# Peacebeuponu94/lachain

Hardware: AMD Instinct MI355X
Metric: BLS12-381 TPKE decryption-share verifications/sec (batched VerifyShare, N=22 F=7) (higher is better)
Workload: dtype u32 (381-bit Montgomery, 12x32-bit limbs); 1 GPU; configs[1]: 1M TPKE decryption shares, N=22 F=7 validators, one MI355X per rank; ciphertexts_per_rank=47663, decryptors=22, degree=7, parallelism=shard1, decision_mismatches=0, batches_in_flight=4, hw_queues=4, hw_queues_env=4

## Files before the change

### include/lachain_bls.h

```cpp
#ifndef LACHAIN_BLS_H
#define LACHAIN_BLS_H
#include <stddef.h>
#include <stdint.h>
#ifdef __cplusplus
extern "C" {
#endif

#define MCL_BLS12_381 5
#define MCLBN_COMPILED_TIME_VAR 46

typedef int64_t mclInt;
typedef size_t mclSize;
typedef struct { uint64_t d[4]; } mclBnFr;
typedef struct { uint64_t d[6]; } mclBnFp;
typedef struct { mclBnFp d[2]; } mclBnFp2;
typedef struct { mclBnFp x, y, z; } mclBnG1;
typedef struct { mclBnFp2 x, y, z; } mclBnG2;
typedef struct { mclBnFp d[12]; } mclBnGT;

int mclBn_init(int curve, int compiledTimeVar);
int mclBn_getOpUnitSize(void);
int mclBn_getG1ByteSize(void);
int mclBn_getFrByteSize(void);
int mclBn_getFpByteSize(void);
// ... 98 lines not shown
int lcb_tpke_encrypt_phase1(uint8_t *u_out, uint8_t *t_out, const uint8_t y[48], const uint8_t *r, size_t n);
int lcb_tpke_encrypt_phase2(uint8_t *w_out, const uint8_t *u, const uint8_t *r, const uint8_t *v_data,
                            const uint32_t *v_off, size_t n);

int lcb_ts_verify_shares(uint8_t *accept, size_t n, const uint8_t *pks, size_t n_pks, const uint8_t *sigs,
                         const uint8_t *msg_data, const uint32_t *msg_off, size_t n_msgs,
                         const uint32_t *msg_idx, const uint32_t *pk_idx);
int lcb_ts_verify_shares_dev(uint8_t *accept, size_t n, const uint8_t *pks, size_t n_pks, const uint8_t *sigs,
                             const uint8_t *msg_data, const uint32_t *msg_off, size_t n_msgs,
                             const uint32_t *msg_idx, const uint32_t *pk_idx, void *stream);

int lcb_ts_prepare_dev(const uint8_t *pks, size_t n_pks, const uint8_t *msg_data, const uint32_t *msg_off,
                       size_t n_msgs, void *stream);
int lcb_ts_verify_prepared_dev(uint8_t *accept, size_t n, size_t n_pks, size_t n_msgs, const uint8_t *sigs,
                               const uint32_t *msg_idx, const uint32_t *pk_idx, void *stream);
int lcb_ts_assemble_dev(uint8_t *sig_out, uint8_t *status, const uint8_t *accept, const uint8_t *sigs,
                        size_t per_round, size_t k, size_t n_rounds, void *stream);

int lcb_tpke_partial_decrypt_prepared_dev(uint8_t *ui_out, uint8_t *status, const uint8_t *x_raw, size_t x_stride,
                                          const uint8_t *cts_u, size_t n_cts, void *stream);
int lcb_tpke_combine_dev(uint8_t *u_out, uint8_t *status, const uint8_t *accept, const uint8_t *shares,
                         size_t per_ct, size_t k, size_t n_cts, void *stream);
int lcb_tpke_combine_ordered_dev(uint8_t *u_out, uint8_t *status, const uint8_t *accept, const uint8_t *shares,
                                 const uint32_t *order, size_t per_ct, size_t k, size_t n_cts, void *stream);
int lcb_ts_assemble_ordered_dev(uint8_t *sig_out, uint8_t *status, const uint8_t *accept, const uint8_t *sigs,
                                const uint32_t *order, size_t per_round, size_t k, size_t n_rounds, void *stream);

int lcb_tpke_verify_phase_ms(float ms[2]);
int lcb_set_lines_coop_max(int max_sets);
int lcb_set_keys_first(int on);
int lcb_set_rlc_share_exponents(int on);
int lcb_set_rlc_lane_permutation(int on);
int lcb_set_rlc_pos_table_min(uint32_t shares_per_key);

int lcb_tpke_verify_prepared_batched_dev(uint8_t *accept, size_t n_shares, size_t n_keys, size_t n_cts,
                                         const uint32_t *ct_idx, const uint32_t *dec_idx, const uint8_t *ui,
                                         void *stream);
int lcb_tpke_verify_shares_batched_dev(uint8_t *accept, size_t n_shares, const uint8_t *y_keys, size_t n_keys,
                                       const uint8_t *cts_u, const uint8_t *cts_w, const uint8_t *v_data,
                                       const uint32_t *v_off, size_t n_cts, const uint32_t *ct_idx,
                                       const uint32_t *dec_idx, const uint8_t *ui, void *stream);
int lcb_tpke_verify_shares_cached(uint8_t *accept, size_t n, const uint8_t *y_keys, size_t n_keys,
                                  const uint8_t *cts_u, const uint8_t *cts_w, const uint8_t *v_data,
                                  const uint32_t *v_off, size_t n_cts, const uint32_t *ct_idx, const uint32_t *dec_idx,
                                  const uint8_t *ui);
int lcb_tpke_verify_shares_batched(uint8_t *accept, size_t n_shares, const uint8_t *y_keys, size_t n_keys,
                                   const uint8_t *cts_u, const uint8_t *cts_w, const uint8_t *v_data,
                                   const uint32_t *v_off, size_t n_cts, const uint32_t *ct_idx,
                                   const uint32_t *dec_idx, const uint8_t *ui);
int lcb_ts_verify_prepared_batched_dev(uint8_t *accept, size_t n, size_t n_pks, size_t n_msgs, const uint8_t *sigs,
                                       const uint32_t *msg_idx, const uint32_t *pk_idx, void *stream);
int lcb_ts_verify_shares_batched_dev(uint8_t *accept, size_t n, const uint8_t *pks, size_t n_pks, const uint8_t *sigs,
                                     const uint8_t *msg_data, const uint32_t *msg_off, size_t n_msgs,
                                     const uint32_t *msg_idx, const uint32_t *pk_idx, void *stream);
int lcb_ts_verify_shares_batched(uint8_t *accept, size_t n, const uint8_t *pks, size_t n_pks, const uint8_t *sigs,
                                 const uint8_t *msg_data, const uint32_t *msg_off, size_t n_msgs,
                                 const uint32_t *msg_idx, const uint32_t *pk_idx);
int lcb_tpke_batched_stats(uint32_t levels[8], float ms[6]);
void lcb_set_batch_seed(const uint8_t *seed32);
void lcb_set_batch_census(size_t min_shares);
int lcb_batched_census(uint32_t out[4]);
int lcb_set_coop_max(uint32_t max_checks);
int lcb_set_coop_miller_max(uint32_t max_checks);
int lcb_set_fe_pair_min(uint32_t min_entries);
int lcb_tpke_fe_pair_stats(uint32_t out[4]);
int lcb_set_busy_coop_max(uint32_t max_checks);
// ... 399 lines not shown
```

### lachain_amd/csrc/k_rlc_rand.hip

```cpp
#include "kcommon.hpp"
#include "rlc_common.hpp"

LCB_ASM_LIBRARY(k_rlc_rand)
LCB_TU_CONFIG(k_rlc_rand)

extern "C" __global__ void LCB_BOUNDS k_rlc_key_tables(const g1a_st *keys, u32 n_keys, u32 *jtab, u32 *pre, u32 *tab,
                                                      uint8_t *ktab_ok) {
    LCB_LATENCY_PRIO();
    u32 t = blockIdx.x * blockDim.x + threadIdx.x;
    if (t >= LCB_KTAB_LANES * n_keys) return;
    u32 k = t / LCB_KTAB_LANES, w = (t / LCB_KTAB_CHUNKS) & 3, ch = t % LCB_KTAB_CHUNKS;
    u32 d0 = ch * LCB_KTAB_CHUNK + 1, d1 = min(255u, d0 + LCB_KTAB_CHUNK - 1);
    g1a K;
    g1a_st ks = keys[k];
    st_to_g1a(K, ks);
    const size_t stride = (size_t)n_keys * LCB_KTAB_ENTRIES;
    const size_t e0 = (size_t)k * LCB_KTAB_ENTRIES + (size_t)w * 255;
    bool ok = ks.ok && !K.inf;
    g1 B, acc;
    jac_from_aff(B, K);
#pragma unroll 1
    for (u32 j = 0; ok && j < 8 * w; j++) jac_dbl(B, B);
    jac_mul_u64_inl(acc, B, d0);
    fp run = fp_one();
// ... 8 lines not shown
    ktab_ok[t] = ok;
    if (!ok) return;
    fp inv, beta;
    fp_inv_gcd(inv, run);
    fp_load_const(beta, LCB_G1_BETA);
#pragma unroll 1
    for (u32 d = d1; d >= d0; d--) {
        g1 p;
        g1_load_soa(p, jtab, stride, e0 + d - 1);
        fp zi, zi2, pd;
        if (d > d0) {
            soa_load<12>(&pd, pre, stride, e0 + d - 2);
            fp_mul(zi, inv, pd);
            fp_mul(inv, inv, p.z);
        } else {
            zi = inv;
        }
        fp_sqr(zi2, zi);
        fp xyb[3];
        fp_mul(xyb[0], p.x, zi2);
        fp_mul(zi2, zi2, zi);
        fp_mul(xyb[1], p.y, zi2);
        fp_mul(xyb[2], xyb[0], beta);
        soa_store<36>(tab, stride, e0 + d - 1, xyb);
    }
}

extern "C" __global__ void __launch_bounds__(LCB_BLOCK) __attribute__((amdgpu_waves_per_eu(1)))
k_tpke_rlc_points(u32 n_cts, const g1a_st *keys, u32 n_keys, const u32 *ct_idx,
                                                       const u32 *dec_idx, const uint8_t *ui, u32 i0, u32 n,
                                                       rlc_key key, u32 *rU, u32 *rY, uint8_t *accept,
                                                       const u32 *ktab, const uint8_t *ktab_ok, const u32 *susp,
                                                       const u32 *perm, const uint8_t *bin, const u32 *P,
                                                       const uint8_t *pinf) {
    const u32 t = blockIdx.x * blockDim.x + threadIdx.x;
    if (t >= n - i0) return;
    u32 i = perm ? perm[t] : i0 + t;
    if (i < i0 || i >= n) return;
    u32 c = ct_idx[i], d = dec_idx[i];
    bool ok = d < n_keys && c < n_cts;
    g1a Ui, Y;
    ok = g1_decompress(Ui, ui + 48 * (size_t)i) && ok;
    g1a_st ks = keys[d < n_keys ? d : 0];
    ok = ok && ks.ok;
    st_to_g1a(Y, ks);
    if (ok && !key_suspect_live(susp, d, n_keys)) {
        u32 a, b;
        const u32 bn = bin ? bin[i] & (RLC_POS_BINS - 1) : 0;
        if (bin) rlc_scalar_dom(key, bn, RLC_DOM_POS, a, b);
        else rlc_scalar(key, i, a, b);
        {
            g1 p;
            g1_mul_ab_wave(p, Ui, a, b);
            g1_store_soa(rU, n, i, p);
        }
        g1 q;
        if (P) {
            const size_t ne = (size_t)RLC_POS_BINS * n_keys, e = (size_t)bn * n_keys + d;
            jac_set_inf(q);
            if (!pinf[e]) {
                soa_load<24>(&q, P, ne, e);
                q.z = fp_one();
            }
        } else if (ktab_usable(ktab_ok, d)) {
            g1_mul_ab_tab(q, ktab, n_keys, d, a, b);
        } else {
            g1_mul_ab_n(q, Y, a, b);
        }
        g1_store_soa(rY, n, i, q);
    } else {
        g1 p;
        jac_set_inf(p);
        g1_store_soa(rU, n, i, p);
        g1_store_soa(rY, n, i, p);
    }
    accept[i] = ok;
}

extern "C" __global__ void LCB_BOUNDS k_tpke_rlc_sum(const uint4 *desc, u32 n_groups, u32 lanes, const uint8_t *ct_ok,
                                                    const uint8_t *ct_g2, const g1a_st *keys, u32 n_keys,
                                                    const u32 *dec_idx, const uint8_t *ui, const u32 *rU,
                                                    const u32 *rY, u32 n, g1a_st *gpts, uint8_t *accept,
                                                    uint8_t *gexact, u32 *wsum, const u32 *susp, uint8_t *cval) {
    LCB_LATENCY_PRIO();
    __shared__ g1 part[LCB_BLOCK];
    const u32 t = blockIdx.x * blockDim.x + threadIdx.x;
// ... 196 lines not shown
}
extern "C" void lcbk_rlc_records_debug(hipStream_t s, const u32 *rA, const u32 *rB, u32 i0, u32 n, int ts,
                                       uint8_t *outA, uint8_t *outB) {
    dim3 grid((n + LCB_BLOCK - 1) / LCB_BLOCK);
    LCB_LAUNCH(k_rlc_records_debug, rA, rB, i0, n, ts ? 1u : 0u, outA, outB);
}
extern "C" void lcbk_ts_rlc_points(hipStream_t s, u32 n_msgs, const void *pks, u32 n_pks, const u32 *msg_idx,
                                   const u32 *pk_idx, const uint8_t *sigs, u32 i0, u32 n, const u32 key[10], u32 *rP,
                                   u32 *rS, uint8_t *accept, void *desc, u32 *count, const u32 *ktab,
                                   const uint8_t *ktab_ok, const u32 *susp, void *dec) {
    rlc_key k;
    for (int j = 0; j < 8; j++) k.k[j] = key[j];
    k.nonce[0] = key[8];
    k.nonce[1] = key[9];
    dim3 grid((n - i0 + LCB_BLOCK - 1) / LCB_BLOCK);
    LCB_LAUNCH(k_ts_rlc_points, n_msgs, (const g1a_st *)pks, n_pks, msg_idx, pk_idx, sigs, i0, n, k, rP, rS, accept,
               (uint4 *)desc, count, ktab, ktab_ok, susp, (ts_share_st *)dec);
}

extern "C" void lcbk_rlc_key_tables(dim3 grid, hipStream_t s, const void *keys, u32 n_keys, u32 *ws, u32 **tab,
                                    uint8_t **ktab_ok) {
    const size_t ne = (size_t)n_keys * LCB_KTAB_ENTRIES;
    u32 *jtab = ws, *pre = ws + 36 * ne, *t = ws + 48 * ne;
    uint8_t *okv = (uint8_t *)(ws + 84 * ne);
    *tab = t;
    *ktab_ok = okv;
    grid = dim3((LCB_KTAB_LANES * n_keys + LCB_BLOCK - 1) / LCB_BLOCK);
    LCB_LAUNCH(k_rlc_key_tables, (const g1a_st *)keys, n_keys, jtab, pre, t, okv);
}
extern "C" void lcbk_tpke_rlc_points(hipStream_t s, u32 n_cts, const void *keys, u32 n_keys, const u32 *ct_idx,
                                     const u32 *dec_idx, const uint8_t *ui, u32 i0, u32 n, const u32 key[10], u32 *rU,
                                     u32 *rY, uint8_t *accept, const u32 *ktab, const uint8_t *ktab_ok,
                                     const u32 *susp, const u32 *perm, const uint8_t *bin, const u32 *P,
                                     const uint8_t *pinf) {
    rlc_key k;
    for (int j = 0; j < 8; j++) k.k[j] = key[j];
    k.nonce[0] = key[8];
    k.nonce[1] = key[9];
    dim3 grid((n - i0 + LCB_BLOCK - 1) / LCB_BLOCK);
    LCB_LAUNCH(k_tpke_rlc_points, n_cts, (const g1a_st *)keys, n_keys, ct_idx, dec_idx, ui, i0, n, k, rU, rY, accept,
               ktab, ktab_ok, susp, perm, bin, bin ? P : nullptr, pinf);
}
extern "C" void lcbk_tpke_rlc_sum(dim3 grid, hipStream_t s, const void *desc, u32 n_groups, u32 lanes,
                                  const uint8_t *ct_ok, const uint8_t *ct_g2, const void *keys, u32 n_keys,
                                  const u32 *dec_idx, const uint8_t *ui, const u32 *rU, const u32 *rY, u32 n,
                                  void *gpts, uint8_t *accept, uint8_t *gexact, u32 *wsum, const u32 *susp,
                                  uint8_t *cval) {
    LCB_LAUNCH(k_tpke_rlc_sum, (const uint4 *)desc, n_groups, lanes, ct_ok, ct_g2, (const g1a_st *)keys, n_keys,
               dec_idx, ui, rU, rY, n, (g1a_st *)gpts, accept, gexact, wsum, susp, cval);
}
extern "C" void lcbk_tpke_rlc_wsum2(hipStream_t s, const void *sdesc, u32 ns, const u32 *open, const u32 *rU,
                                    const u32 *rY, u32 n, const u32 *dec_idx, u32 n_keys, const u32 *susp, void *gpts,
                                    void *sdesc_out) {
    if (!ns) return;
    dim3 grid((2 * (size_t)ns + LCB_BLOCK - 1) / LCB_BLOCK);
    LCB_LAUNCH(k_tpke_rlc_wsum2, (const uint4 *)sdesc, ns, open, rU, rY, n, dec_idx, n_keys, susp, (g1a_st *)gpts,
               (uint4 *)sdesc_out);
}
```

### lachain_amd/csrc/launch.h

```cpp
#pragma once
#include <hip/hip_runtime.h>
#include <stdint.h>
#include "ops.h"
typedef uint32_t u32;
#define LCB_TS_SHARE_REC_BYTES 304
extern "C" void lcbk_g1_decompress(dim3 grid, hipStream_t s, const uint8_t *in, u32 n, void *out);
extern "C" void lcbk_g2_decompress(dim3 grid, hipStream_t s, const uint8_t *in, u32 n, void *out);
extern "C" void lcbk_tpke_ct_prepare(dim3 grid, hipStream_t s, const uint8_t *cts_u, const uint8_t *cts_w, const uint8_t *v_data, const u32 *v_off, u32 n_cts, u32 *lines, uint8_t *ct_ok, int orig_cof, const u32 *slot);
extern "C" void lcbk_tpke_ct_prepare_w64(hipStream_t s, const uint8_t *cts_u, const uint8_t *cts_w, const uint8_t *v_data, const u32 *v_off, u32 n_cts, u32 *lines, uint8_t *ct_ok, int orig_cof);
extern "C" void lcbk_tpke_ct_prepare_h(hipStream_t s, const uint8_t *cts_u, const uint8_t *v_data, const u32 *v_off, u32 c0, u32 c1, u32 *lines, uint8_t *h_ok, int flags);
extern "C" void lcbk_tpke_ct_prepare_w(hipStream_t s, const uint8_t *cts_u, const uint8_t *cts_w, u32 c0, u32 c1, u32 *lines, uint8_t *ct_ok, uint8_t *w_g2, int flags);
extern "C" void lcbk_tpke_ct_prepare_hw(hipStream_t s, const uint8_t *cts_u, const uint8_t *cts_w, const uint8_t *v_data, const u32 *v_off, u32 n_cts, u32 *lines, uint8_t *h_ok, uint8_t *ct_ok, uint8_t *w_g2, int flags);
extern "C" void lcbk_ct_ok_merge(hipStream_t s, uint8_t *ct_ok, const uint8_t *h_ok, u32 c0, u32 c1);
extern "C" void lcbk_lineset_fill(dim3 grid, hipStream_t s, u32 *lines, u32 n_sets, const u32 *sets, uint8_t *w_g2);
extern "C" void lcbk_mcl_g2_hash(hipStream_t s, u32 *io, int orig_cof);
extern "C" size_t lcbk_h2g2_debug_in_words(void);
extern "C" size_t lcbk_h2g2_debug_out_words(void);
extern "C" int lcbk_h2g2_debug_ops(void);
extern "C" void lcbk_h2g2_debug(hipStream_t s, int op, const u32 *in, u32 n, u32 *out);
extern "C" void lcbk_mcl_g2_clear(hipStream_t s, u32 *io);
extern "C" void lcbk_lineset_coop(hipStream_t s, u32 *lines, u32 n_sets, const u32 *sets, uint8_t *w_g2);
extern "C" void lcbk_lineset_coop_2w(hipStream_t s, u32 *lines, u32 n_sets, const u32 *sets, uint8_t *w_g2);
extern "C" void lcbk_tpke_miller(dim3 grid, hipStream_t s, const u32 *lines, const uint8_t *ct_ok, u32 n_cts, const void *keys, u32 n_keys, const u32 *ct_idx, const u32 *dec_idx, const uint8_t *ui, u32 n, u32 *f_soa, uint8_t *accept);
extern "C" int lcbk_fe_slots();
// ... 67 lines not shown
extern "C" void lcbk_secp_sign(hipStream_t s, const uint8_t *hashes, const uint8_t *privs, const uint8_t *nonces, u32 n, const void *g_table, int chain_id, int use_new, uint8_t *out, uint8_t *ok);
extern "C" size_t lcbk_secp_rjob_bytes(void);
extern "C" size_t lcbk_secp_rpoint_bytes(void);
extern "C" void lcbk_secp_rec_scalars(hipStream_t s, const uint8_t *hashes, const uint8_t *sigs, u32 sig_len, u32 want_len, int chain_id, int special, u32 n, void *jobs);
extern "C" void lcbk_secp_recover(hipStream_t s, const void *jobs, u32 n, const void *g_table, void *pts);
extern "C" size_t lcbk_secp_debug_in_words(void);
extern "C" size_t lcbk_secp_debug_out_words(void);
extern "C" int lcbk_secp_debug_ops(void);
extern "C" void lcbk_secp_debug(hipStream_t s, int op, const u32 *a, const u32 *b, u32 n, u32 *out);
extern "C" void lcbk_secp_rec_finish(hipStream_t s, const void *pts, u32 n, uint8_t *pub33, uint8_t *addr20, uint8_t *ok, const uint8_t *from20, uint8_t *accept);
extern "C" void lcbk_keccak256(hipStream_t s, const uint8_t *data, const uint64_t *off, u32 n, uint8_t *out32);
extern "C" void lcbk_tx_hash(hipStream_t s, const uint8_t *txs, const uint8_t *inv, const uint64_t *off, const uint8_t *sigs, u32 sig_len, const uint8_t *claimed, u32 chain_id, u32 n, uint8_t *raw32, uint8_t *full32, uint8_t *match, uint32_t *long_ws);
extern "C" void lcbk_tx_detail(hipStream_t s, const uint8_t *match, const uint8_t *rec_ok, const uint8_t *addr20, const uint8_t *txs, u32 n, uint8_t *accept, uint8_t *detail);
extern "C" void lcbk_tx_root_ok(hipStream_t s, const uint8_t *roots, const uint8_t *expected, u32 n, uint8_t *root_ok);
extern "C" void lcbk_rawtx_decode(hipStream_t s, const uint8_t *raw, const uint64_t *off, uint64_t span_base, u32 sig_len, u32 chain_id, u32 n, uint8_t *status, uint8_t *detail, uint8_t *txs, uint64_t *span, uint8_t *sigs, uint8_t *raw32, uint8_t *full32, uint32_t *long_ws);
extern "C" void lcbk_rawtx_finish(hipStream_t s, const uint8_t *status, const uint8_t *rec_ok, const uint8_t *addr20, const uint8_t *det_in, u32 n, uint8_t *accept, uint8_t *detail, uint8_t *txs);
extern "C" void lcbk_trie_flat(hipStream_t s, const uint8_t *nodes, const uint8_t *data, const uint64_t *off, const uint8_t *expected32, u32 n, uint8_t *out32, uint8_t *accept, uint32_t *list_ws);
extern "C" void lcbk_trie_level(hipStream_t s, uint8_t *hashes32, const uint8_t *nodes, const uint8_t *data, const uint64_t *off, const uint64_t *child_off, const int64_t *child_ref, const uint8_t *literals32, const uint64_t *order, u32 count);
extern "C" size_t lcbk_trie_root_ws_bytes(u32 n, u32 B);
extern "C" int lcbk_trie_roots(hipStream_t s, uint8_t *roots32, uint8_t *status, const uint8_t *keys, const uint64_t *key_off, const uint8_t *values, const uint64_t *val_off, const uint64_t *trie_off, u32 B, u32 n, int keys_hashed, void *ws);
extern "C" void lcbk_kdf_xor(hipStream_t s, uint8_t *out, const uint8_t *seeds, const uint32_t *seed_off, const uint8_t *data, const uint32_t *data_off, const uint8_t *ok, u32 n);
extern "C" void lcbk_kdf_xor_strided(hipStream_t s, uint8_t *out, const uint8_t *seeds, u32 seed_stride, const uint8_t *data, const uint32_t *data_off, const uint8_t *ok, u32 n);
extern "C" void lcbk_tpke_ids_to_x(hipStream_t s, const int32_t *ids, u32 ne, uint8_t *xs);
extern "C" size_t lcbk_ecdh_job_bytes(void);
extern "C" size_t lcbk_ecdh_point_bytes(void);
extern "C" void lcbk_ecdh_scalars(hipStream_t s, const uint8_t *pub, const uint64_t *off, u32 min_len, const uint8_t *scalars32, const u32 *idx, u32 n_scalars, u32 n, void *jobs);
extern "C" void lcbk_ecdh_mul(hipStream_t s, const void *jobs, u32 n, void *pts);
extern "C" void lcbk_ecdh_finish(hipStream_t s, const void *pts, u32 n, uint8_t *key32, uint8_t *ok);
extern "C" void lcbk_gcm_offsets(hipStream_t s, const uint64_t *off, u32 n, u32 overhead, uint64_t *out_off);
extern "C" void lcbk_gcm_encrypt(hipStream_t s, const uint8_t *keys32, const uint8_t *nonces16, const uint8_t *pt, const uint64_t *pt_off, u32 n, uint8_t *out, const uint8_t *hdr33, const uint8_t *ok_in);
extern "C" void lcbk_gcm_decrypt(hipStream_t s, const uint8_t *keys32, const uint8_t *ct, const uint64_t *ct_off, const uint64_t *out_off, u32 n, u32 hdr, uint8_t *pt_out, uint8_t *ok_out, const uint8_t *ok_in);
extern "C" size_t lcbk_key_table_bytes(u32 n_keys);
extern "C" void lcbk_rlc_key_tables(dim3 grid, hipStream_t s, const void *keys, u32 n_keys, u32 *ws, u32 **tab, uint8_t **ktab_ok);
extern "C" void lcbk_tpke_rlc_points(hipStream_t s, u32 n_cts, const void *keys, u32 n_keys, const u32 *ct_idx, const u32 *dec_idx, const uint8_t *ui, u32 i0, u32 n, const u32 key[10], u32 *rU, u32 *rY, uint8_t *accept, const u32 *ktab, const uint8_t *ktab_ok, const u32 *susp, const u32 *perm, const uint8_t *bin, const u32 *P, const uint8_t *pinf);
extern "C" size_t lcbk_rlc_pos_bins_bytes(void);
extern "C" void lcbk_rlc_positions(hipStream_t s, const u32 *ct_idx, u32 i0, u32 n, u32 n_cts, uint8_t *bin, u32 *bins, u32 *perm);
extern "C" size_t lcbk_rlc_pos_table_bytes(u32 n_keys);
extern "C" void lcbk_rlc_pos_table(hipStream_t s, const void *keys, u32 n_keys, const u32 key[10], const u32 *ktab, const uint8_t *ktab_ok, u32 *ws, u32 **P, uint8_t **pinf);
extern "C" void lcbk_ts_rlc_points(hipStream_t s, u32 n_msgs, const void *pks, u32 n_pks, const u32 *msg_idx, const u32 *pk_idx, const uint8_t *sigs, u32 i0, u32 n, const u32 key[10], u32 *rP, u32 *rS, uint8_t *accept, void *desc, u32 *count, const u32 *ktab, const uint8_t *ktab_ok, const u32 *susp, void *dec);
extern "C" void lcbk_rlc_scalars_debug(hipStream_t s, const u32 *key10, const u32 *ctr, const u32 *dom, u32 n, u32 *ab);
extern "C" void lcbk_rlc_records_debug(hipStream_t s, const u32 *rA, const u32 *rB, u32 i0, u32 n, int ts, uint8_t *outA, uint8_t *outB);
extern "C" void lcbk_rlc_groups(hipStream_t s, const u32 *key_idx, u32 i0, u32 n, u32 n_keys, u32 cap, void *desc, u32 *count);
extern "C" void lcbk_tpke_rlc_sum(dim3 grid, hipStream_t s, const void *desc, u32 n_groups, u32 lanes, const uint8_t *ct_ok, const uint8_t *ct_g2, const void *keys, u32 n_keys, const u32 *dec_idx, const uint8_t *ui, const u32 *rU, const u32 *rY, u32 n, void *gpts, uint8_t *accept, uint8_t *gexact, u32 *wsum, const u32 *susp, uint8_t *cval);
extern "C" void lcbk_tpke_rlc_wsum(dim3 grid, hipStream_t s, const void *sdesc, u32 n_s, const u32 *wsum, u32 n_l1, void *gpts);
extern "C" void lcbk_tpke_rlc_miller(dim3 grid, hipStream_t s, const u32 *lines, const void *desc, const void *gpts, u32 n_groups, u32 *f_soa, uint8_t *gacc);
extern "C" void lcbk_ts_rlc_sum(dim3 grid, hipStream_t s, const void *desc, u32 n_groups, u32 first, const uint8_t *msg_ok, const void *pks, u32 n_pks, const u32 *pk_idx, const uint8_t *sigs, const u32 *rP, const u32 *rS, u32 n, void *gpts, uint8_t *accept, uint8_t *gexact, u32 *wsum, const u32 *susp, uint8_t *cval);
extern "C" void lcbk_ts_rlc_wsum(dim3 grid, hipStream_t s, const void *sdesc, u32 n_s, const u32 *wsum, u32 n_l1, void *gpts);
extern "C" void lcbk_ts_rlc_miller(dim3 grid, hipStream_t s, const u32 *lines, const void *desc, const void *gpts, u32 n_groups, u32 *f_soa, uint8_t *gacc);
extern "C" void lcbk_rlc_resolve(dim3 grid, hipStream_t s, const void *desc, u32 o, u32 m, const uint8_t *gacc, const uint8_t *gexact, const u32 *park, u32 first, uint8_t *accept, void *next, u32 *next_count, void *search, u32 *search_count, u32 *gamma, const u32 *key_idx, u32 n_keys, const u32 *susp);
extern "C" void lcbk_tpke_rlc_wsum2(hipStream_t s, const void *sdesc, u32 ns, const u32 *open, const u32 *rU, const u32 *rY, u32 n, const u32 *dec_idx, u32 n_keys, const u32 *susp, void *gpts, void *sdesc_out);
extern "C" void lcbk_rlc_park_copy(hipStream_t s, const u32 *park, u32 o, u32 m, u32 *dst, const u32 *map);
extern "C" void lcbk_tpke_rlc_search2a(hipStream_t s, const void *search, u32 ns, const u32 *gamma0, const u32 *gamma12, uint8_t *accept, u32 *open, u32 *open_count);
extern "C" int lcbk_search2b_by_position(void);
extern "C" int lcbk_search2b_debug(void *p);
extern "C" void lcbk_tpke_rlc_search2b(hipStream_t s, const void *search, u32 ns, u32 n_open, const u32 *gamma0, const u32 *gamma12, const u32 *open, const u32 *open_count, uint8_t *accept, void *next, u32 *next_count, const u32 *key_idx, u32 n_keys, const u32 *susp);
extern "C" void lcbk_tpke_rlc_search2b_asm(hipStream_t s, const void *search, u32 ns, u32 n_open, const u32 *gamma0, const u32 *gamma12, const u32 *open, const u32 *open_count, uint8_t *accept, void *next, u32 *next_count, const u32 *key_idx, u32 n_keys, const u32 *susp, u32 *park);
extern "C" size_t lcbk_tpke_rlc_search2b_asm_park_bytes(u32 n_open);
extern "C" void lcbk_fe_pair_pack(hipStream_t s, const void *desc, const u32 *f, u32 m, u32 *park, u32 jobs, uint8_t *kind, uint8_t *pacc, u32 by_set);
extern "C" void lcbk_fe_pair_list(hipStream_t s, const uint8_t *kind, const uint8_t *pacc, u32 jobs, u32 *list, u32 *p2idx, u32 *cnt);
extern "C" void lcbk_fe_pair_gather(hipStream_t s, const u32 *f, u32 m, const u32 *list, u32 n2, u32 *park2, uint8_t *pacc2);
extern "C" void lcbk_fe_pair_finish(hipStream_t s, u32 *f, u32 m, u32 *park, u32 jobs, const uint8_t *kind, const uint8_t *pacc, const u32 *p2idx, const u32 *park2, u32 n2, uint8_t *gacc);
extern "C" void lcbk_rlc_search(dim3 grid, hipStream_t s, const void *search, u32 o, u32 m, const u32 *gamma, const u32 *park, uint8_t *accept, void *next, u32 *next_count, const u32 *key_idx, u32 n_keys, const u32 *susp);
extern "C" void lcbk_rlc_census_desc(hipStream_t s, const u32 *grp_idx, const u32 *key_idx, u32 m, u32 n_grp, u32 n_keys, void *desc, uint8_t *accept);
extern "C" void lcbk_rlc_census_stats(hipStream_t s, const u32 *key_idx, u32 m, u32 n_keys, const uint8_t *cval, const uint8_t *accept, u32 *susp, u32 *count);
extern "C" void lcbk_rlc_suspect_split(hipStream_t s, const void *desc, u32 n_groups, const u32 *key_idx, u32 n_keys, const u32 *susp, const uint8_t *accept, void *out, u32 *count);
extern "C" size_t lcbk_ts_grp_bytes();
extern "C" void lcbk_coop_tpke_miller(hipStream_t s, const u32 *lines, const void *desc, const void *gpts, u32 n_groups, u32 *f_soa, uint8_t *gacc, uint8_t *fb, u32 npairs, int fallback);
// ... 86 lines not shown
```

### lachain_amd/csrc/lcb_batch.cpp

```cpp
#include <hip/hip_runtime.h>
#include <string.h>
#include <stdio.h>
#include <stdlib.h>
#include <mutex>
#include <atomic>
#include <vector>
#include <algorithm>
#include <sys/random.h>

#include "launch.h"
#include "lcb_internal.hpp"
#include "../../include/lachain_bls.h"

using namespace lcb_int;

#define LCB_RLC_GROUP_CAP 32
#define LCB_VERIFY_CHUNK (c->chunk)
#ifndef LCB_SEARCH2B_ASM
#define LCB_SEARCH2B_ASM 1
#endif

std::atomic<uint32_t> lcb_int::g_coop_max{32768};

namespace {
// ... 106 lines not shown
    w.dB = (uint8_t *)c->rlc[RLC_DESC_B].get(n * 16);
    w.cnt = (u32 *)c->rlc[RLC_CNT].get(32);
    const size_t sw = (n_keys + 31) / 32;
    w.susp = m ? (u32 *)c->rlc[RLC_SUSP].get(4 * sw) : nullptr;
    w.m = m;
    if (!w.rA || !w.rB || !w.dA || !w.dB || !w.cnt || (m && !w.susp)) { set_err("device allocation failed"); return false; }
    if (!c->rlc_ev_ready) {
        for (auto &e : c->rlc_ev) hipEventCreate(&e);
        for (auto &e : c->rlc_lev_ev) hipEventCreate(&e);
        c->rlc_ev_ready = true;
    }
    hipMemsetAsync(w.cnt, 0, 32, s);
    if (m) hipMemsetAsync(w.susp, 0, 4 * sw, s);
    c->rlc_census[CENSUS_SHARES] = m;
    c->prep_timed = false;
    c->rlc_census[CENSUS_SUSPECTS] = c->rlc_census[CENSUS_GROUPS] = c->rlc_census[CENSUS_ENTRIES] = 0;
    return true;
}
u32 *rlc_key_tables(lcb_ctx *c, const void *keys, size_t n_keys, hipStream_t s, uint8_t **ktab_ok) {
    *ktab_ok = nullptr;
    if (!n_keys || n_keys > 4096) return nullptr;
    u32 *ws = (u32 *)c->rlc[RLC_KTAB].get(lcbk_key_table_bytes((u32)n_keys));
    if (!ws) return nullptr;
    u32 *tab = nullptr;
    lcbk_rlc_key_tables(dim3(1), s, keys, (u32)n_keys, ws, &tab, ktab_ok);
    return tab;
}
long tuning_env(const char *name, long dflt) {
    const char *e = getenv(name);
    return (e && *e && env_on("LCB_ALLOW_TUNING")) ? atol(e) : dflt;
}
std::atomic<int> g_share_exp{tuning_env("LCB_RLC_SHARE_EXP", 0) ? 1 : 0};
std::atomic<int> g_lane_perm{tuning_env("LCB_RLC_LANE_PERM", 1) ? 1 : 0};
#ifndef LCB_POS_TABLE_MIN
#define LCB_POS_TABLE_MIN 512u
#endif
std::atomic<uint32_t> g_pos_table_min{(uint32_t)tuning_env("LCB_RLC_POS_TABLE_MIN", LCB_POS_TABLE_MIN)};
int rlc_points_enqueue(lcb_ctx *c, RlcWs &w, uint8_t *d_accept, size_t n, size_t n_keys, size_t n_cts,
                       const uint32_t *d_ct, const uint32_t *d_dec, const uint8_t *d_ui, hipStream_t s) {
    u32 key[10];
    if (!rlc_key_fill(c, key)) return -1;
    rlc_note_records(c, RLC_TPKE, n, w.m);
    const bool pos = !g_share_exp.load(), permute = g_lane_perm.load() != 0;
    c->rlc_pos_exp = pos;
    hipEventRecord(c->rlc_ev[0], s);
    if (w.m < n) {
        uint8_t *kok = w.kok;
        u32 *ktab = w.ktab_pre ? w.ktab : rlc_key_tables(c, c->t_keys.p, n_keys, s, &kok);
        uint8_t *bin = nullptr, *pinf = nullptr;
        u32 *perm = nullptr, *P = nullptr;
        if (pos || permute) {
            bin = (uint8_t *)c->rlc[RLC_POS_BIN].get(n);
            u32 *bins = (u32 *)c->rlc[RLC_POS_BINS].get(lcbk_rlc_pos_bins_bytes());
            if (permute) perm = (u32 *)c->rlc[RLC_POS_PERM].get(4 * (n - w.m));
            if (!bin || !bins || (permute && !perm)) { set_err("device allocation failed (positions)"); return -1; }
            lcbk_rlc_positions(s, d_ct, w.m, (u32)n, (u32)n_cts, bin, bins, perm);
        }
        const uint32_t tmin = g_pos_table_min.load();
        if (pos && ktab && tmin != UINT32_MAX && n - w.m >= (size_t)tmin * n_keys) {
            u32 *pws = (u32 *)c->rlc[RLC_POS_TABLE].get(lcbk_rlc_pos_table_bytes((u32)n_keys));
            if (!pws) { set_err("device allocation failed (position table)"); return -1; }
            lcbk_rlc_pos_table(s, c->t_keys.p, (u32)n_keys, key, ktab, kok, pws, &P, &pinf);
        }
        lcbk_tpke_rlc_points(s, (u32)n_cts, c->t_keys.p, (u32)n_keys, d_ct, d_dec, d_ui, w.m, (u32)n, key, w.rA, w.rB,
                             d_accept, ktab, kok, w.susp, perm, pos ? bin : nullptr, P, pinf);
        static_assert(LCB_RLC_GROUP_CAP == 32, "the position bins hold the level-1 groups' cap (rlc_common.hpp RLC_POS_CAP)");
        lcbk_rlc_groups(s, d_ct, w.m, (u32)n, (u32)n_cts, LCB_RLC_GROUP_CAP, w.dA, w.cnt + CNT_GROUPS);
    }
    hipEventRecord(c->rlc_ev[1], s);
    return launch_ok("tpke batched verify launch") ? 0 : -1;
}
int ts_rlc_points_enqueue(lcb_ctx *c, RlcWs &w, uint8_t *d_accept, size_t n, size_t n_pks, size_t n_msgs,
                          const uint8_t *d_sigs, const uint32_t *d_midx, const uint32_t *d_pidx, hipStream_t s) {
    u32 key[10];
    if (!rlc_key_fill(c, key)) return -1;
    rlc_note_records(c, RLC_TS, n, w.m);
    hipEventRecord(c->rlc_ev[0], s);
    if (w.m < n) {
        uint8_t *kok = w.kok;
        u32 *ktab = w.ktab_pre ? w.ktab : rlc_key_tables(c, c->s_keys.p, n_pks, s, &kok);
        const size_t rec = n * (size_t)LCB_TS_SHARE_REC_BYTES;
        const bool grow = c->s_dec.cap < rec;
        void *dec = c->s_dec.get(rec);
        if (dec && grow) hipMemsetAsync(dec, 0, c->s_dec.cap, s);
        c->s_dec_n = dec ? c->s_dec.cap / LCB_TS_SHARE_REC_BYTES : 0;
        lcbk_ts_rlc_points(s, (u32)n_msgs, c->s_keys.p, (u32)n_pks, d_midx, d_pidx, d_sigs, w.m, (u32)n, key, w.rA,
                           w.rB, d_accept, w.dA, w.cnt + CNT_GROUPS, ktab, kok, w.susp, dec);
        lcbk_rlc_groups(s, d_midx, w.m, (u32)n, (u32)n_msgs, 128, w.dA, w.cnt + CNT_GROUPS);
    }
    hipEventRecord(c->rlc_ev[1], s);
    return launch_ok("ts batched verify launch") ? 0 : -1;
}
bool read_counts(u32 *v, const u32 *d, int k, hipStream_t s) {
    if (hipMemcpyAsync(v, d, 4 * k, hipMemcpyDeviceToHost, s) != hipSuccess || hipStreamSynchronize(s) != hipSuccess) {
        set_err("batched verify: group count");
        return false;
    }
    return true;
// ... 734 lines not shown
}
extern "C" int lcb_set_fe_pair_min(uint32_t min_entries) {
    if (!tuning_allowed("lcb_set_fe_pair_min")) return -1;
    g_fe_pair_min.store(min_entries);
    return 0;
}
extern "C" int lcb_set_busy_coop_max(uint32_t max_checks) {
    if (!tuning_allowed("lcb_set_busy_coop_max")) return -1;
    g_busy_coop_max.store(max_checks);
    return 0;
}
extern "C" uint32_t lcb_busy_coop_max(void) { return g_busy_coop_max.load(); }
extern "C" int lcb_set_level_mode(int mode) {
    if (!tuning_allowed("lcb_set_level_mode")) return -1;
    if (mode < 0 || mode > 2) { set_err("lcb_set_level_mode: 0 (by the count), 1 (never busy), 2 (always busy)"); return -1; }
    g_level_mode.store(mode);
    return 0;
}
extern "C" int lcb_set_fork_mode(int mode) {
    if (!tuning_allowed("lcb_set_fork_mode")) return -1;
    g_fork_mode.store(mode >= 1 && mode <= 4 ? mode : 0);
    return 0;
}
extern "C" int lcb_set_rlc_share_exponents(int on) {
    if (!tuning_allowed("lcb_set_rlc_share_exponents")) return -1;
    g_share_exp.store(on ? 1 : 0);
    return 0;
}
extern "C" int lcb_set_rlc_lane_permutation(int on) {
    if (!tuning_allowed("lcb_set_rlc_lane_permutation")) return -1;
    g_lane_perm.store(on ? 1 : 0);
    return 0;
}
extern "C" int lcb_set_rlc_pos_table_min(uint32_t shares_per_key) {
    if (!tuning_allowed("lcb_set_rlc_pos_table_min")) return -1;
    g_pos_table_min.store(shares_per_key);
    return 0;
}
extern "C" int lcb_set_keys_first(int on) {
    if (!tuning_allowed("lcb_set_keys_first")) return -1;
    g_keys_first.store(on ? 1 : 0);
    return 0;
}
```

### lachain_amd/csrc/rlc_common.hpp

```cpp
#pragma once
#include "kcommon.hpp"

struct rlc_key { u32 k[8]; u32 nonce[2]; };

#define LCB_RLC_SINGLES 8

DI bool key_suspect(const u32 *susp, u32 k, u32 n_keys) {
    return susp && k < n_keys && ((susp[k >> 5] >> (k & 31)) & 1u);
}
DI bool key_suspect_live(const u32 *susp, u32 k, u32 n_keys) {
    if (!susp || k >= n_keys) return false;
    return (__atomic_load_n(susp + (k >> 5), __ATOMIC_RELAXED) >> (k & 31)) & 1u;
}

DI u32 rotl32(u32 x, int r) { return (x << r) | (x >> (32 - r)); }
#define CHACHA_QR(a, b, c, d)                  \
    a += b; d ^= a; d = rotl32(d, 16);         \
    c += d; b ^= c; b = rotl32(b, 12);         \
    a += b; d ^= a; d = rotl32(d, 8);          \
    c += d; b ^= c; b = rotl32(b, 7);
#define RLC_DOM_POS 1u
#define RLC_POS_CAP 32u
#define RLC_POS_SETS 4u
#define RLC_POS_BINS (RLC_POS_SETS * RLC_POS_CAP)
DI void rlc_scalar_dom(const rlc_key &key, u32 ctr, u32 dom, u32 &a, u32 &b) {
    u32 x[16], s[16];
    s[0] = 0x61707865u; s[1] = 0x3320646eu; s[2] = 0x79622d32u; s[3] = 0x6b206574u;
#pragma unroll
    for (int j = 0; j < 8; j++) s[4 + j] = key.k[j];
    s[12] = ctr; s[13] = dom; s[14] = key.nonce[0]; s[15] = key.nonce[1];
#pragma unroll
    for (int j = 0; j < 16; j++) x[j] = s[j];
#pragma unroll 1
    for (int r = 0; r < 10; r++) {
// ... 68 lines not shown
    if (P.inf) return;
#if LCB_AB_LEAN
    fp bx, beta;
    fp_load_const(beta, LCB_G1_BETA);
    fp_mul(bx, P.x, beta);
#pragma unroll 1
    for (int k = 31; k >= 0; k--) {
        jac_dbl(r, r);
        u32 da = (a >> k) & 1, db = (b >> k) & 1;
        if (da | db) {
            fp ax, ay;
            if (da & db) {
                fp_add(ax, P.x, bx);
                fp_neg(ax, ax);
                fp_neg(ay, P.y);
            } else {
                ax = da ? P.x : bx;
                ay = P.y;
            }
            jac_add_aff(r, r, ax, ay);
        }
    }
#else
    fp bx, b2x, ny;
    g1_ab_addends(bx, b2x, ny, P);
#pragma unroll 1
    for (int k = 31; k >= 0; k--) {
        jac_dbl(r, r);
        u32 da = (a >> k) & 1, db = (b >> k) & 1;
        if (da | db) jac_add_aff(r, r, da ? (db ? b2x : P.x) : bx, (da & db) ? ny : P.y);
    }
#endif
}
DI void g1_mul_ab_wave(g1 &r, const g1a &P, u32 a, u32 b) {
    if (P.inf) { jac_set_inf(r); return; }
    const u32 a0 = (u32)__builtin_amdgcn_readfirstlane((int)a), b0 = (u32)__builtin_amdgcn_readfirstlane((int)b);
    if (__ballot(a != a0 || b != b0) == 0) g1_mul_ab_inl(r, P, a0, b0);
    else g1_mul_ab_inl(r, P, a, b);
}
DI void g2_mul_ab_inl(g2 &r, const g2a &S, u32 a, u32 b) {
    jac_set_inf(r);
    if (S.inf) return;
#if LCB_AB_LEAN
    fp2 x2;
    {
        fp beta;
        fp_load_const(beta, LCB_G1_BETA);
        fp2_mul_fp(x2, S.x, beta);
    }
#pragma unroll 1
    for (int k = 31; k >= 0; k--) {
        jac_dbl(r, r);
        u32 da = (a >> k) & 1, db = (b >> k) & 1;
        if (da | db) {
            fp2 ax, ay;
            if (da & db) {
                ax = x2;
                fp2_neg(ay, S.y);
            } else if (da) {
                ax = S.x;
                ay = S.y;
            } else {
                fp2_add(ax, S.x, x2);
                fp2_neg(ax, ax);
                ay = S.y;
            }
            jac_add_aff(r, r, ax, ay);
        }
    }
#else
    fp2 x4, x2, ny;
// ... 158 lines not shown
```

### lachain_amd/native.py

```python
import ctypes
import os
import struct
import threading
from typing import NamedTuple, Optional

_HERE = os.path.dirname(os.path.abspath(__file__))
LIB_PATH = os.environ.get("LCB_LIB_PATH") or os.path.join(_HERE, "liblachain_bls.so")
MCL_BLS12_381 = 5
MCLBN_COMPILED_TIME_VAR = 46

_lib = None
_lock = threading.Lock()

c_u8p = ctypes.POINTER(ctypes.c_uint8)
c_u32p = ctypes.POINTER(ctypes.c_uint32)
c_u64p = ctypes.POINTER(ctypes.c_uint64)
c_size = ctypes.c_size_t


class mclBnFr(ctypes.Structure):
    _fields_ = [("d", ctypes.c_uint64 * 4)]


class mclBnFp(ctypes.Structure):
# ... 4 lines not shown
    _fields_ = [("d", mclBnFp * 2)]


class mclBnG1(ctypes.Structure):
    _fields_ = [("x", mclBnFp), ("y", mclBnFp), ("z", mclBnFp)]


class mclBnG2(ctypes.Structure):
    _fields_ = [("x", mclBnFp2), ("y", mclBnFp2), ("z", mclBnFp2)]


class mclBnGT(ctypes.Structure):
    _fields_ = [("d", mclBnFp * 12)]


_SIGS = {
    "mclBn_init": (ctypes.c_int, [ctypes.c_int, ctypes.c_int]),
    "lcb_set_device": (ctypes.c_int, [ctypes.c_int]),
    "lcb_get_device": (ctypes.c_int, []),
    "lcb_set_original_g2_cofactor": (None, [ctypes.c_int]),
    "lcb_set_line_mode": (ctypes.c_int, [ctypes.c_int]),
    "lcb_set_g2_sign_from_b": (ctypes.c_int, [ctypes.c_int]),
    "lcb_set_msm_chunk": (ctypes.c_int, [ctypes.c_int]),
    "lcb_set_msm_segments": (ctypes.c_int, [ctypes.c_int]),
    "lcb_set_wave_priority": (ctypes.c_int, [ctypes.c_int]),
    "lcb_last_error": (ctypes.c_char_p, []),
    "lcb_error_count": (ctypes.c_uint64, []),
    "lcb_test_inject_failure": (ctypes.c_int, [ctypes.c_int, ctypes.c_int]),
    "lcb_set_lines_coop_max": (ctypes.c_int, [ctypes.c_int]),
    "lcb_set_keys_first": (ctypes.c_int, [ctypes.c_int]),
    "lcb_set_rlc_share_exponents": (ctypes.c_int, [ctypes.c_int]),
    "lcb_set_rlc_lane_permutation": (ctypes.c_int, [ctypes.c_int]),
    "lcb_set_rlc_pos_table_min": (ctypes.c_int, [ctypes.c_uint32]),
    "lcb_test_linesets": (ctypes.c_int, [ctypes.c_int, ctypes.c_char_p, ctypes.c_char_p, ctypes.c_size_t,
                                          ctypes.c_void_p, ctypes.c_void_p]),
    "lcb_tpke_verify_shares": (ctypes.c_int, [c_u8p, c_size, c_u8p, c_size, c_u8p, c_u8p, c_u8p, c_u32p, c_size,
                                              c_u32p, c_u32p, c_u8p]),
    "lcb_tpke_verify_shares_cached": (ctypes.c_int, [c_u8p, c_size, c_u8p, c_size, c_u8p, c_u8p, c_u8p, c_u32p, c_size,
                                                     c_u32p, c_u32p, c_u8p]),
    "lcb_tpke_verify_shares_dev": (ctypes.c_int, [ctypes.c_void_p, c_size, ctypes.c_void_p, c_size, ctypes.c_void_p,
                                                  ctypes.c_void_p, ctypes.c_void_p, ctypes.c_void_p, c_size,
                                                  ctypes.c_void_p, ctypes.c_void_p, ctypes.c_void_p, ctypes.c_void_p]),
    "lcb_tpke_prepare_dev": (ctypes.c_int, [ctypes.c_void_p, c_size, ctypes.c_void_p, ctypes.c_void_p, ctypes.c_void_p,
                                            ctypes.c_void_p, c_size, ctypes.c_void_p]),
    "lcb_tpke_verify_prepared_dev": (ctypes.c_int, [ctypes.c_void_p, c_size, c_size, c_size, ctypes.c_void_p,
                                                    ctypes.c_void_p, ctypes.c_void_p, ctypes.c_void_p]),
    "lcb_tpke_verify_shares_batched": (ctypes.c_int, [c_u8p, c_size, c_u8p, c_size, c_u8p, c_u8p, c_u8p, c_u32p,
                                                      c_size, c_u32p, c_u32p, c_u8p]),
    "lcb_tpke_verify_shares_batched_dev": (ctypes.c_int, [ctypes.c_void_p, c_size, ctypes.c_void_p, c_size,
                                                          ctypes.c_void_p, ctypes.c_void_p, ctypes.c_void_p,
                                                          ctypes.c_void_p, c_size, ctypes.c_void_p, ctypes.c_void_p,
                                                          ctypes.c_void_p, ctypes.c_void_p]),
    "lcb_tpke_verify_prepared_batched_dev": (ctypes.c_int, [ctypes.c_void_p, c_size, c_size, c_size, ctypes.c_void_p,
                                                            ctypes.c_void_p, ctypes.c_void_p, ctypes.c_void_p]),
    "lcb_ts_verify_shares_batched": (ctypes.c_int, [c_u8p, c_size, c_u8p, c_size, c_u8p, c_u8p, c_u32p, c_size,
                                                    c_u32p, c_u32p]),
    "lcb_ts_verify_prepared_batched_dev": (ctypes.c_int, [ctypes.c_void_p, c_size, c_size, c_size, ctypes.c_void_p,
                                                          ctypes.c_void_p, ctypes.c_void_p, ctypes.c_void_p]),
    "lcb_ts_verify_shares_batched_dev": (ctypes.c_int, [ctypes.c_void_p, c_size, ctypes.c_void_p, c_size,
                                                        ctypes.c_void_p, ctypes.c_void_p, ctypes.c_void_p, c_size,
                                                        ctypes.c_void_p, ctypes.c_void_p, ctypes.c_void_p]),
    "lcb_tpke_batched_stats": (ctypes.c_int, [ctypes.POINTER(ctypes.c_uint32), ctypes.POINTER(ctypes.c_float)]),
    "lcb_set_batch_seed": (None, [ctypes.c_char_p]),
    "lcb_set_batch_census": (None, [c_size]),
    "lcb_set_coop_max": (ctypes.c_int, [ctypes.c_uint32]),
    "lcb_set_fe_pair_min": (ctypes.c_int, [ctypes.c_uint32]),
# ... 1181 lines not shown

def test_linesets(points, coop, force=None):
    import numpy as np
    n = len(points)
    force = bytes(force) if force is not None else bytes(n)
    out = np.zeros((n, 6592), dtype=np.uint32)
    g2f = np.zeros(max(1, n // 2), dtype=np.uint8)
    mode = coop if isinstance(coop, int) and not isinstance(coop, bool) else (1 if coop else 0)
    if lib().lcb_test_linesets(mode, b"".join(points), force, n, out.ctypes.data, g2f.ctypes.data) != 0:
        raise RuntimeError("test_linesets: " + last_error())
    return out, g2f[: n // 2]


def set_lines_coop_max(max_sets):
    _tuning(lib().lcb_set_lines_coop_max(int(max_sets)), "set_lines_coop_max")


def set_keys_first(on):
    _tuning(lib().lcb_set_keys_first(1 if on else 0), "set_keys_first")


def set_rlc_share_exponents(on):
    _tuning(lib().lcb_set_rlc_share_exponents(1 if on else 0), "set_rlc_share_exponents")


def set_rlc_lane_permutation(on):
    _tuning(lib().lcb_set_rlc_lane_permutation(1 if on else 0), "set_rlc_lane_permutation")


def set_rlc_pos_table_min(shares_per_key):
    _tuning(lib().lcb_set_rlc_pos_table_min(int(shares_per_key)), "set_rlc_pos_table_min")


def set_wave_priority(on):
    _tuning(lib().lcb_set_wave_priority(1 if on else 0), "set_wave_priority")


def set_msm_segments(max_segments):
    _tuning(lib().lcb_set_msm_segments(int(max_segments)), "set_msm_segments")


def set_msm_chunk(records_per_lane):
    _tuning(lib().lcb_set_msm_chunk(int(records_per_lane)), "set_msm_chunk")


def set_scratch_gate(nbytes):
    _tuning(lib().lcb_set_scratch_gate(int(nbytes)), "set_scratch_gate")


def scratch_info():
    out = (ctypes.c_uint64 * 6)()
    if lib().lcb_scratch_info(out) != 0:
        raise RuntimeError("lcb_scratch_info failed")
    keys = ("pool", "bind_limit", "slots", "queues", "per_queue", "threshold")
    return dict(zip(keys, (int(v) for v in out)))


def scratch_gate_stats():
    a, b = ctypes.c_uint64(), ctypes.c_uint64()
    lib().lcb_scratch_gate_stats(ctypes.byref(a), ctypes.byref(b))
    return a.value, b.value


def set_persist_blocks(max_blocks):
    _tuning(lib().lcb_set_persist_blocks(int(max_blocks)), "set_persist_blocks")

# ... 181 lines not shown
```

Baseline: 19.08 million share verifications/s.

## Use joint sparse form recoding for wave-uniform RLC G1 double-scalar multiplication

Adds a joint sparse form (JSF) signed-digit recoding of the two 32-bit random scalars (a, b) and a new G1 multiply path. It precomputes P, the endomorphism image beta*P and the combined point P±beta*P in a shared-Z affine form, then runs a double-and-add over the sparser signed digits. The goal is fewer point additions per RLC share point than the existing unsigned interleaved method. It only runs when the scalars are uniform across the wave (the positional-bin path). It stores the precomputed combined point and its Z factor into the rU buffer as scratch, reloads them inside the loop, then overwrites them with the result. Default on via LCB_RLC_SIGNED_DIGITS.

```diff
diff --git a/include/lachain_bls.h b/include/lachain_bls.h
--- a/include/lachain_bls.h
+++ b/include/lachain_bls.h
@@ -154,6 +154,7 @@
 int lcb_set_rlc_share_exponents(int on);
 int lcb_set_rlc_lane_permutation(int on);
 int lcb_set_rlc_pos_table_min(uint32_t shares_per_key);
+int lcb_set_rlc_signed_digits(int on);
 
 int lcb_tpke_verify_prepared_batched_dev(uint8_t *accept, size_t n_shares, size_t n_keys, size_t n_cts,
                                          const uint32_t *ct_idx, const uint32_t *dec_idx, const uint8_t *ui,
diff --git a/lachain_amd/csrc/k_rlc_rand.hip b/lachain_amd/csrc/k_rlc_rand.hip
--- a/lachain_amd/csrc/k_rlc_rand.hip
+++ b/lachain_amd/csrc/k_rlc_rand.hip
@@ -64,7 +64,7 @@
                                                        rlc_key key, u32 *rU, u32 *rY, uint8_t *accept,
                                                        const u32 *ktab, const uint8_t *ktab_ok, const u32 *susp,
                                                        const u32 *perm, const uint8_t *bin, const u32 *P,
-                                                       const uint8_t *pinf) {
+                                                       const uint8_t *pinf, u32 jsf) {
     const u32 t = blockIdx.x * blockDim.x + threadIdx.x;
     if (t >= n - i0) return;
     u32 i = perm ? perm[t] : i0 + t;
@@ -83,7 +83,7 @@
         else rlc_scalar(key, i, a, b);
         {
             g1 p;
-            g1_mul_ab_wave(p, Ui, a, b);
+            g1_mul_ab_wave(p, Ui, a, b, jsf != 0, rU, n, i);
             g1_store_soa(rU, n, i, p);
         }
         g1 q;
@@ -346,14 +346,14 @@
                                      const u32 *dec_idx, const uint8_t *ui, u32 i0, u32 n, const u32 key[10], u32 *rU,
                                      u32 *rY, uint8_t *accept, const u32 *ktab, const uint8_t *ktab_ok,
                                      const u32 *susp, const u32 *perm, const uint8_t *bin, const u32 *P,
-                                     const uint8_t *pinf) {
+                                     const uint8_t *pinf, int signed_digits) {
     rlc_key k;
     for (int j = 0; j < 8; j++) k.k[j] = key[j];
     k.nonce[0] = key[8];
     k.nonce[1] = key[9];
     dim3 grid((n - i0 + LCB_BLOCK - 1) / LCB_BLOCK);
     LCB_LAUNCH(k_tpke_rlc_points, n_cts, (const g1a_st *)keys, n_keys, ct_idx, dec_idx, ui, i0, n, k, rU, rY, accept,
-               ktab, ktab_ok, susp, perm, bin, bin ? P : nullptr, pinf);
+               ktab, ktab_ok, susp, perm, bin, bin ? P : nullptr, pinf, signed_digits ? 1u : 0u);
 }
 extern "C" void lcbk_tpke_rlc_sum(dim3 grid, hipStream_t s, const void *desc, u32 n_groups, u32 lanes,
                                   const uint8_t *ct_ok, const uint8_t *ct_g2, const void *keys, u32 n_keys,
diff --git a/lachain_amd/csrc/launch.h b/lachain_amd/csrc/launch.h
--- a/lachain_amd/csrc/launch.h
+++ b/lachain_amd/csrc/launch.h
@@ -123,7 +123,7 @@
 extern "C" void lcbk_gcm_decrypt(hipStream_t s, const uint8_t *keys32, const uint8_t *ct, const uint64_t *ct_off, const uint64_t *out_off, u32 n, u32 hdr, uint8_t *pt_out, uint8_t *ok_out, const uint8_t *ok_in);
 extern "C" size_t lcbk_key_table_bytes(u32 n_keys);
 extern "C" void lcbk_rlc_key_tables(dim3 grid, hipStream_t s, const void *keys, u32 n_keys, u32 *ws, u32 **tab, uint8_t **ktab_ok);
-extern "C" void lcbk_tpke_rlc_points(hipStream_t s, u32 n_cts, const void *keys, u32 n_keys, const u32 *ct_idx, const u32 *dec_idx, const uint8_t *ui, u32 i0, u32 n, const u32 key[10], u32 *rU, u32 *rY, uint8_t *accept, const u32 *ktab, const uint8_t *ktab_ok, const u32 *susp, const u32 *perm, const uint8_t *bin, const u32 *P, const uint8_t *pinf);
+extern "C" void lcbk_tpke_rlc_points(hipStream_t s, u32 n_cts, const void *keys, u32 n_keys, const u32 *ct_idx, const u32 *dec_idx, const uint8_t *ui, u32 i0, u32 n, const u32 key[10], u32 *rU, u32 *rY, uint8_t *accept, const u32 *ktab, const uint8_t *ktab_ok, const u32 *susp, const u32 *perm, const uint8_t *bin, const u32 *P, const uint8_t *pinf, int signed_digits);
 extern "C" size_t lcbk_rlc_pos_bins_bytes(void);
 extern "C" void lcbk_rlc_positions(hipStream_t s, const u32 *ct_idx, u32 i0, u32 n, u32 n_cts, uint8_t *bin, u32 *bins, u32 *perm);
 extern "C" size_t lcbk_rlc_pos_table_bytes(u32 n_keys);
diff --git a/lachain_amd/csrc/lcb_batch.cpp b/lachain_amd/csrc/lcb_batch.cpp
--- a/lachain_amd/csrc/lcb_batch.cpp
+++ b/lachain_amd/csrc/lcb_batch.cpp
@@ -162,6 +162,7 @@
 }
 std::atomic<int> g_share_exp{tuning_env("LCB_RLC_SHARE_EXP", 0) ? 1 : 0};
 std::atomic<int> g_lane_perm{tuning_env("LCB_RLC_LANE_PERM", 1) ? 1 : 0};
+std::atomic<int> g_signed_digits{tuning_env("LCB_RLC_SIGNED_DIGITS", 1) ? 1 : 0};
 #ifndef LCB_POS_TABLE_MIN
 #define LCB_POS_TABLE_MIN 512u
 #endif
@@ -193,7 +194,7 @@
             lcbk_rlc_pos_table(s, c->t_keys.p, (u32)n_keys, key, ktab, kok, pws, &P, &pinf);
         }
         lcbk_tpke_rlc_points(s, (u32)n_cts, c->t_keys.p, (u32)n_keys, d_ct, d_dec, d_ui, w.m, (u32)n, key, w.rA, w.rB,
-                             d_accept, ktab, kok, w.susp, perm, pos ? bin : nullptr, P, pinf);
+                             d_accept, ktab, kok, w.susp, perm, pos ? bin : nullptr, P, pinf, g_signed_digits.load());
         static_assert(LCB_RLC_GROUP_CAP == 32, "the position bins hold the level-1 groups' cap (rlc_common.hpp RLC_POS_CAP)");
         lcbk_rlc_groups(s, d_ct, w.m, (u32)n, (u32)n_cts, LCB_RLC_GROUP_CAP, w.dA, w.cnt + CNT_GROUPS);
     }
@@ -994,6 +995,11 @@
     g_lane_perm.store(on ? 1 : 0);
     return 0;
 }
+extern "C" int lcb_set_rlc_signed_digits(int on) {
+    if (!tuning_allowed("lcb_set_rlc_signed_digits")) return -1;
+    g_signed_digits.store(on ? 1 : 0);
+    return 0;
+}
 extern "C" int lcb_set_rlc_pos_table_min(uint32_t shares_per_key) {
     if (!tuning_allowed("lcb_set_rlc_pos_table_min")) return -1;
     g_pos_table_min.store(shares_per_key);
diff --git a/lachain_amd/csrc/rlc_common.hpp b/lachain_amd/csrc/rlc_common.hpp
--- a/lachain_amd/csrc/rlc_common.hpp
+++ b/lachain_amd/csrc/rlc_common.hpp
@@ -1,5 +1,6 @@
 #pragma once
 #include "kcommon.hpp"
+#include "rlc_jsf.hpp"
 
 struct rlc_key { u32 k[8]; u32 nonce[2]; };
 
@@ -134,11 +135,72 @@
     }
 #endif
 }
-DI void g1_mul_ab_wave(g1 &r, const g1a &P, u32 a, u32 b) {
+DI void g1_mul_ab_jsf(g1 &r, const g1a &P, u32 a, u32 b, u32 *rec, size_t n, size_t i) {
+    rlc_jsf j;
+    rlc_jsf_recode(j, a, b);
+    const u64 nz = j.nz_a | j.nz_b;
+    jac_set_inf(r);
+    if (!nz) return;
+    fp x, y, bx;
+    {
+        fp beta, t;
+        g1 st;
+        fp_load_const(beta, LCB_G1_BETA);
+        fp_mul(bx, P.x, beta);
+        fp_sub(st.z, bx, P.x);
+        fp_sqr(t, st.z);
+        fp_mul(x, P.x, t);
+        fp_mul(t, t, st.z);
+        fp_mul(y, P.y, t);
+        fp_mul(bx, x, beta);
+        fp_sqr(t, P.y);
+        fp_add(t, t, t);
+        fp_add(t, t, t);
+        fp_add(st.x, x, bx);
+        fp_sub(st.x, t, st.x);
+        fp_sub(t, st.x, x);
+        fp_mul(t, t, P.y);
+        fp_add(t, t, t);
+        fp_sub(st.y, t, y);
+        g1_store_soa(rec, n, i, st);
+    }
+    const int top = 63 - __builtin_clzll(nz);
+#pragma unroll 1
+    for (int k = top; k >= 0; k--) {
+        if (k != top) jac_dbl(r, r);
+        if (!((nz >> k) & 1)) continue;
+        const bool da = (j.nz_a >> k) & 1, db = (j.nz_b >> k) & 1, sa = (j.neg_a >> k) & 1, sb = (j.neg_b >> k) & 1;
+        fp ax, ay;
+        bool neg;
+        if (da && db && sa != sb) {
+            asm volatile("" ::: "memory");
+            soa_load<12>(&ax, rec, n, i);
+            soa_load<12>(&ay, rec + (size_t)12 * n, n, i);
+            neg = sa;
+        } else if (da && db) {
+            fp_add(ax, x, bx);
+            fp_neg(ax, ax);
+            ay = y;
+            neg = !sa;
+        } else {
+            ax = da ? x : bx;
+            ay = y;
+            neg = da ? sa : sb;
+        }
+        if (neg) fp_neg(ay, ay);
+        jac_add_aff(r, r, ax, ay);
+    }
+    fp h;
+    asm volatile("" ::: "memory");
+    soa_load<12>(&h, rec + (size_t)24 * n, n, i);
+    fp_mul(r.z, r.z, h);
+}
+DI void g1_mul_ab_wave(g1 &r, const g1a &P, u32 a, u32 b, bool jsf, u32 *rec, size_t n, size_t i) {
     if (P.inf) { jac_set_inf(r); return; }
     const u32 a0 = (u32)__builtin_amdgcn_readfirstlane((int)a), b0 = (u32)__builtin_amdgcn_readfirstlane((int)b);
-    if (__ballot(a != a0 || b != b0) == 0) g1_mul_ab_inl(r, P, a0, b0);
-    else g1_mul_ab_inl(r, P, a, b);
+    if (__ballot(a != a0 || b != b0) != 0) g1_mul_ab_inl(r, P, a, b);
+    else if (!jsf || __ballot(fp_is_zero(P.x)) != 0) g1_mul_ab_inl(r, P, a0, b0);
+    else g1_mul_ab_jsf(r, P, a0, b0, rec, n, i);
 }
 DI void g2_mul_ab_inl(g2 &r, const g2a &S, u32 a, u32 b) {
     jac_set_inf(r);
diff --git a/lachain_amd/csrc/rlc_jsf.hpp b/lachain_amd/csrc/rlc_jsf.hpp
--- /dev/null
+++ b/lachain_amd/csrc/rlc_jsf.hpp
@@ -0,0 +1,41 @@
+#pragma once
+#include <stdint.h>
+
+#if defined(__HIPCC__) || defined(__CUDACC__)
+#define RLC_JSF_FN __host__ __device__ inline
+#else
+#define RLC_JSF_FN inline
+#endif
+
+#define RLC_JSF_COLS 33
+
+struct rlc_jsf {
+    uint64_t nz_a, neg_a;
+    uint64_t nz_b, neg_b;
+};
+
+RLC_JSF_FN int rlc_jsf_digit(uint64_t l, uint64_t m) {
+    if (!(l & 1)) return 0;
+    int u = 2 - (int)(l & 3);
+    if (((l & 7) == 3 || (l & 7) == 5) && (m & 3) == 2) u = -u;
+    return u;
+}
+
+RLC_JSF_FN void rlc_jsf_recode(rlc_jsf &o, uint32_t a, uint32_t b) {
+    uint64_t k0 = a, k1 = b;
+    uint32_t d0 = 0, d1 = 0;
+    o.nz_a = o.neg_a = o.nz_b = o.neg_b = 0;
+    for (int j = 0; j < RLC_JSF_COLS; j++) {
+        const uint64_t l0 = k0 + d0, l1 = k1 + d1;
+        if (!(l0 | l1)) break;
+        const int u0 = rlc_jsf_digit(l0, l1), u1 = rlc_jsf_digit(l1, l0);
+        if (2 * (int)d0 == 1 + u0) d0 = 1 - d0;
+        if (2 * (int)d1 == 1 + u1) d1 = 1 - d1;
+        k0 >>= 1;
+        k1 >>= 1;
+        o.nz_a |= (uint64_t)(u0 != 0) << j;
+        o.neg_a |= (uint64_t)(u0 < 0) << j;
+        o.nz_b |= (uint64_t)(u1 != 0) << j;
+        o.neg_b |= (uint64_t)(u1 < 0) << j;
+    }
+}
diff --git a/lachain_amd/native.py b/lachain_amd/native.py
--- a/lachain_amd/native.py
+++ b/lachain_amd/native.py
@@ -60,6 +60,7 @@
     "lcb_set_rlc_share_exponents": (ctypes.c_int, [ctypes.c_int]),
     "lcb_set_rlc_lane_permutation": (ctypes.c_int, [ctypes.c_int]),
     "lcb_set_rlc_pos_table_min": (ctypes.c_int, [ctypes.c_uint32]),
+    "lcb_set_rlc_signed_digits": (ctypes.c_int, [ctypes.c_int]),
     "lcb_test_linesets": (ctypes.c_int, [ctypes.c_int, ctypes.c_char_p, ctypes.c_char_p, ctypes.c_size_t,
                                           ctypes.c_void_p, ctypes.c_void_p]),
     "lcb_tpke_verify_shares": (ctypes.c_int, [c_u8p, c_size, c_u8p, c_size, c_u8p, c_u8p, c_u8p, c_u32p, c_size,
@@ -1307,6 +1308,10 @@
     _tuning(lib().lcb_set_rlc_pos_table_min(int(shares_per_key)), "set_rlc_pos_table_min")
 
 
+def set_rlc_signed_digits(on):
+    _tuning(lib().lcb_set_rlc_signed_digits(1 if on else 0), "set_rlc_signed_digits")
+
+
 def set_wave_priority(on):
     _tuning(lib().lcb_set_wave_priority(1 if on else 0), "set_wave_priority")
 
```

After: 19.58 million share verifications/s (median of 6 runs). +2.6%, better.
